# fishaudio/fish-diffusion

Hardware: NVIDIA H100
Metric: mel_frames_per_sec_100step_ddpm (higher is better)
Workload: dtype f32 (3x fp16 split-product wgmma, fp32 accumulate)

## Files before the change

### fish_diffusion_b200/csrc/fd_tapgemm_tc.cu

```cuda
#include <cuda.h>
#include "fd_common.cuh"
#include "fd_host.h"
#include "fd_tc_ptx.cuh"

namespace {

constexpr int BLOCK_M = 128;

constexpr int ring_stages(int stage_bytes, int bias_floats) {
  return fd_tc_ring_stages(1024  + bias_floats * 4 + 2 * FD_TC_MAX_STAGES * 8 + FD_TC_SCRATCH_BYTES,
                           stage_bytes);
}

template <int BLOCK_N, int BLOCK_K, int EPI, int NPL>
struct Cfg {
  static constexpr bool PP = EPI == FD_EPI_GATE || EPI == FD_EPI_RES_SKIP;
  static constexpr int ROWS = PP ? 64 : BLOCK_M;
  static constexpr int A_BYTES = ROWS * BLOCK_K * 2;
  static constexpr int W_BYTES = BLOCK_N * BLOCK_K * 2;
  static constexpr int GROUP = BLOCK_K >= 64 || PP ? 1 : 64 / BLOCK_K;
  static constexpr int SUB_BYTES = NPL * (A_BYTES + W_BYTES);
  static constexpr int STAGE_BYTES = GROUP * SUB_BYTES;
  static constexpr int TX_BYTES = SUB_BYTES;
  static constexpr int SWIZZLE_BYTES = BLOCK_K * 2;
  static constexpr uint32_t SWIZZLE_MODE = swizzle_mode_for(SWIZZLE_BYTES);
  static constexpr uint32_t SBO = 8 * SWIZZLE_BYTES;
  static constexpr int BIAS_FLOATS = (EPI == FD_EPI_GATE ? 3 : 1) * BLOCK_N;
  static constexpr int BIAS_TOTAL = (PP ? 2 : 1) * BIAS_FLOATS;
  static constexpr int NUM_STAGES = ring_stages(STAGE_BYTES, BIAS_TOTAL);
  static constexpr int SMEM_BYTES = 1024  + NUM_STAGES * STAGE_BYTES + BIAS_TOTAL * 4 +
                                    2 * NUM_STAGES * 8 + FD_TC_SCRATCH_BYTES;
  static_assert(NUM_STAGES >= 2, "pipeline needs at least two stages");
  static_assert(SMEM_BYTES <= FD_TC_SMEM_BUDGET, "shared memory");
};

template <int BLOCK_N, int EPI>
__device__ __forceinline__ void stage_bias(const FdTapGemm& p, int b, int n0, float* bias_s, int i0, int step) {
  if (EPI == FD_EPI_GATE) {
    const size_t bo = (size_t)b * p.gbias_bstride + n0;
    for (int i = i0; i < BLOCK_N; i += step) {
      bias_s[i] = p.gbias_full[bo + i];
      bias_s[BLOCK_N + i] = p.gbias_lo[bo + i];
      bias_s[2 * BLOCK_N + i] = p.gbias_hi[bo + i];
    }
  } else {
    for (int i = i0; i < BLOCK_N; i += step)
      bias_s[i] = p.bias ? p.bias[(size_t)b * p.bias_bstride + n0 + i] : 0.f;
  }
}
template <int EPI>
__device__ __forceinline__ long long bias_key(const FdTapGemm& p, int b, int n0) {
  return EPI == FD_EPI_GATE ? (long long)b * p.gbias_bstride + n0 : (long long)b * p.bias_bstride + n0;
}

template <int BLOCK_N, int EPI, int PREC>
__device__ __forceinline__ void tile_epilogue(const FdTapGemm& p, const float* acc, int b, int n_tile, int rw0,
                                              const float* bias_s, uint32_t my_scratch, int lane) {
  const int n0 = n_tile * BLOCK_N;
  if (EPI == FD_EPI_GATE || EPI == FD_EPI_MAG) {
    constexpr int HALF = BLOCK_N / 2;
    const uint32_t sb = smem_u32(bias_s);
    const int r = lane >> 1, sub = lane & 1;
    const int t = rw0 + r;
    const bool valid = t < p.T;
    const bool e_lo = t < p.dil, e_hi = t + p.dil >= p.T;
    const bool edge_any = __any_sync(0xffffffffu, valid && (e_lo || e_hi));
    const size_t zplane = (size_t)p.B * p.T * p.C, zrow = ((size_t)b * p.T + t) * p.C + (size_t)n_tile * HALF;
    const size_t yplane = (size_t)p.B * p.T * p.n_total, yrow = ((size_t)b * p.T + t) * p.n_total;
    const int halfg = p.gate_tile / 2;
#pragma unroll
    for (int c = 0; c < HALF; c += 16) {
      frag_to_scratch<16>(my_scratch, acc, c, 0, lane);
      frag_to_scratch<16>(my_scratch, acc, HALF + c, 16, lane);
      __syncwarp();
      float g[8], f[8];
      {
        const float4 g0 = scratch_ld4(my_scratch, r, 2 * sub), g1 = scratch_ld4(my_scratch, r, 2 * sub + 1);
        const float4 f0 = scratch_ld4(my_scratch, r, 4 + 2 * sub), f1 = scratch_ld4(my_scratch, r, 5 + 2 * sub);
        g[0] = g0.x; g[1] = g0.y; g[2] = g0.z; g[3] = g0.w; g[4] = g1.x; g[5] = g1.y; g[6] = g1.z; g[7] = g1.w;
        f[0] = f0.x; f[1] = f0.y; f[2] = f0.z; f[3] = f0.w; f[4] = f1.x; f[5] = f1.y; f[6] = f1.z; f[7] = f1.w;
      }
      __syncwarp();
      const int cc = c + 8 * sub;
      if (valid) {
        if (EPI == FD_EPI_MAG) {
          fd_epi_mag<8, PREC>(p, b, t, n_tile * HALF + cc, g, f);
        } else {
          float yg[8], yf[8], z[8];
          {
            float4 c0, c1, d0, d1;
            if (p.addend != nullptr) {
              const float* ad = p.addend + yrow + n0 + cc;
              c0 = __ldcs(reinterpret_cast<const float4*>(ad));
              c1 = __ldcs(reinterpret_cast<const float4*>(ad + 4));
              d0 = __ldcs(reinterpret_cast<const float4*>(ad + HALF));
              d1 = __ldcs(reinterpret_cast<const float4*>(ad + HALF + 4));
            }
            const float4 a0 = lds128(sb + 4u * cc), a1 = lds128(sb + 4u * cc + 16u);
            const float4 b0 = lds128(sb + 4u * (HALF + cc)), b1 = lds128(sb + 4u * (HALF + cc) + 16u);
            const float bg[8] = {a0.x, a0.y, a0.z, a0.w, a1.x, a1.y, a1.z, a1.w};
            const float bf[8] = {b0.x, b0.y, b0.z, b0.w, b1.x, b1.y, b1.z, b1.w};
#pragma unroll
            for (int i = 0; i < 8; ++i) {
              yg[i] = g[i] * p.acc_scale + bg[i];
              yf[i] = f[i] * p.acc_scale + bf[i];
            }
            if (p.addend != nullptr) {
              const float cg[8] = {c0.x, c0.y, c0.z, c0.w, c1.x, c1.y, c1.z, c1.w};
              const float cf[8] = {d0.x, d0.y, d0.z, d0.w, d1.x, d1.y, d1.z, d1.w};
#pragma unroll
              for (int i = 0; i < 8; ++i) { yg[i] += cg[i]; yf[i] += cf[i]; }
            }
          }
          if (edge_any) {
#pragma unroll
            for (int e = 0; e < 2; ++e) {
              if (e == 0 ? e_lo : e_hi) {
                const uint32_t eb = sb + 4u * ((1 + e) * BLOCK_N + cc);
                const float4 a0 = lds128(eb), a1 = lds128(eb + 16u);
                const float4 b0 = lds128(eb + 4u * HALF), b1 = lds128(eb + 4u * HALF + 16u);
                const float eg[8] = {a0.x, a0.y, a0.z, a0.w, a1.x, a1.y, a1.z, a1.w};
                const float ef[8] = {b0.x, b0.y, b0.z, b0.w, b1.x, b1.y, b1.z, b1.w};
#pragma unroll
                for (int i = 0; i < 8; ++i) { yg[i] -= eg[i]; yf[i] -= ef[i]; }
              }
            }
          }
#pragma unroll
          for (int i = 0; i < 8; ++i) z[i] = fd_sigmoid(yg[i]) * fd_tanh(yf[i]);
          if (p.y_planes != nullptr) {
            const int zc0 = n_tile * HALF + cc;
            const int ng = p.gate_tile == BLOCK_N ? n_tile * BLOCK_N + cc : (zc0 / halfg) * p.gate_tile + (zc0 % halfg);
            fd_store_planes<8>(p.y_planes, yplane, yrow + ng, yg, PREC);
            fd_store_planes<8>(p.y_planes, yplane, yrow + ng + halfg, yf, PREC);
          }
          fd_store_planes<8>(p.out_planes, zplane, zrow + cc, z, PREC);
        }
      }
    }
  } else if (BLOCK_N >= 64) {
    const uint32_t bias_addr = smem_u32(bias_s);
    const int j4 = (lane & 7) * 4, rsub = lane >> 3;
    const int rbase = rw0 + rsub;
    const int nrows = rbase < p.T ? min(4, (p.T - rbase + 3) / 4) : 0;
    const uint32_t rowbase = (uint32_t)b * (uint32_t)p.T;
#pragma unroll
    for (int c = 0; c < BLOCK_N; c += 32) {
      const int col = c + j4;
      const int n = n0 + col;
      frag_to_scratch<32>(my_scratch, acc, c, 0, lane);
      __syncwarp();
      float4 a[4];
#pragma unroll
      for (int pp = 0; pp < 4; ++pp) a[pp] = scratch_ld4(my_scratch, 4 * pp + rsub, lane & 7);
      __syncwarp();
      if (EPI == FD_EPI_GATE_BWD) {
        const int half_g = p.gate_tile / 2;
        const uint32_t pg = (uint32_t)((n / half_g) * p.gate_tile + (n % half_g));
        const uint32_t W2 = 2u * (uint32_t)p.C;
        const size_t yplane = (size_t)p.B * p.T * W2;
        const uint16_t* const y_lo = p.y_planes + yplane;
        uint16_t* const o_lo = p.out_planes + yplane;
        float sg4[4] = {0.f, 0.f, 0.f, 0.f}, sf4[4] = {0.f, 0.f, 0.f, 0.f};
        float e0g[4] = {0.f, 0.f, 0.f, 0.f}, e0f[4] = {0.f, 0.f, 0.f, 0.f}, e1g[4] = {0.f, 0.f, 0.f, 0.f}, e1f[4] = {0.f, 0.f, 0.f, 0.f};
        uint2 gh[4], gl[4], fh[4], fl[4];
        uint32_t eo4[4];
#pragma unroll
        for (int pp = 0; pp < 4; ++pp) {
          eo4[pp] = (rowbase + (uint32_t)min(rbase + pp * 4, p.T - 1)) * W2 + pg;
          gh[pp] = *reinterpret_cast<const uint2*>(p.y_planes + eo4[pp]);
          gl[pp] = *reinterpret_cast<const uint2*>(y_lo + eo4[pp]);
          fh[pp] = *reinterpret_cast<const uint2*>(p.y_planes + eo4[pp] + half_g);
          fl[pp] = *reinterpret_cast<const uint2*>(y_lo + eo4[pp] + half_g);
        }
#pragma unroll
        for (int pp = 0; pp < 4; ++pp) {
          if (pp >= nrows) break;
          float g[4], f[4];
          fd_combine2(gh[pp].x, gl[pp].x, PREC, g[0], g[1]);
          fd_combine2(gh[pp].y, gl[pp].y, PREC, g[2], g[3]);
          fd_combine2(fh[pp].x, fl[pp].x, PREC, f[0], f[1]);
          fd_combine2(fh[pp].y, fl[pp].y, PREC, f[2], f[3]);
          const float dzv[4] = {a[pp].x * p.acc_scale, a[pp].y * p.acc_scale, a[pp].z * p.acc_scale, a[pp].w * p.acc_scale};
          float dg[4], df[4];
#pragma unroll
          for (int i = 0; i < 4; ++i) fd_dgate(dzv[i], g[i], f[i], dg[i], df[i]);
          uint32_t h0, l0, h1, l1;
          fd_split2(dg[0], dg[1], PREC, h0, l0);
          fd_split2(dg[2], dg[3], PREC, h1, l1);
          *reinterpret_cast<uint2*>(p.out_planes + eo4[pp]) = make_uint2(h0, h1);
          *reinterpret_cast<uint2*>(o_lo + eo4[pp]) = make_uint2(l0, l1);
          fd_split2(df[0], df[1], PREC, h0, l0);
          fd_split2(df[2], df[3], PREC, h1, l1);
          *reinterpret_cast<uint2*>(p.out_planes + eo4[pp] + half_g) = make_uint2(h0, h1);
          *reinterpret_cast<uint2*>(o_lo + eo4[pp] + half_g) = make_uint2(l0, l1);
          if (p.cs != nullptr) {
            const int tt = rbase + pp * 4;
            const bool in0 = tt < p.dil, in1 = tt + p.dil >= p.T;
#pragma unroll
            for (int i = 0; i < 4; ++i) {
              sg4[i] += dg[i]; sf4[i] += df[i];
              if (in0) { e0g[i] += dg[i]; e0f[i] += df[i]; }
              if (in1) { e1g[i] += dg[i]; e1f[i] += df[i]; }
            }
          }
        }
        if (p.cs != nullptr) {
          const bool edge0 = rw0 < p.dil, edge1 = rw0 + 16 + p.dil > p.T;
#pragma unroll
          for (int i = 0; i < 4; ++i) {
            sg4[i] += __shfl_xor_sync(0xffffffffu, sg4[i], 8); sg4[i] += __shfl_xor_sync(0xffffffffu, sg4[i], 16);
            sf4[i] += __shfl_xor_sync(0xffffffffu, sf4[i], 8); sf4[i] += __shfl_xor_sync(0xffffffffu, sf4[i], 16);
            if (edge0) {
              e0g[i] += __shfl_xor_sync(0xffffffffu, e0g[i], 8); e0g[i] += __shfl_xor_sync(0xffffffffu, e0g[i], 16);
              e0f[i] += __shfl_xor_sync(0xffffffffu, e0f[i], 8); e0f[i] += __shfl_xor_sync(0xffffffffu, e0f[i], 16);
            }
            if (edge1) {
              e1g[i] += __shfl_xor_sync(0xffffffffu, e1g[i], 8); e1g[i] += __shfl_xor_sync(0xffffffffu, e1g[i], 16);
              e1f[i] += __shfl_xor_sync(0xffffffffu, e1f[i], 8); e1f[i] += __shfl_xor_sync(0xffffffffu, e1f[i], 16);
            }
          }
          if (rsub == 0) {
            float* const csb = p.cs + (size_t)b * W2 + pg;
#pragma unroll
            for (int i = 0; i < 4; ++i) {
              atomicAdd(csb + i, sg4[i] * p.cs_scale);
              atomicAdd(csb + half_g + i, sf4[i] * p.cs_scale);
            }
            if (p.cs_edge != nullptr && (edge0 || edge1)) {
              float* const ce0 = p.cs_edge + (size_t)b * W2 + pg;
              float* const ce1 = ce0 + (size_t)p.B * W2;
#pragma unroll
              for (int i = 0; i < 4; ++i) {
                if (edge0) { atomicAdd(ce0 + i, e0g[i] * p.cs_scale); atomicAdd(ce0 + half_g + i, e0f[i] * p.cs_scale); }
                if (edge1) { atomicAdd(ce1 + i, e1g[i] * p.cs_scale); atomicAdd(ce1 + half_g + i, e1f[i] * p.cs_scale); }
              }
            }
          }
        }
      } else if (EPI == FD_EPI_RES_SKIP) {
        const float4 bias4 = lds128(bias_addr + 4u * col);
        const bool is_res = n0 < p.C;
        const uint32_t cn = (uint32_t)(is_res ? n : n - p.C);
        const size_t plane = (size_t)p.B * p.T * p.C;
        uint32_t eo[4];
#pragma unroll
        for (int pp = 0; pp < 4; ++pp)
          eo[pp] = (rowbase + (uint32_t)min(rbase + pp * 4, p.T - 1)) * (uint32_t)p.C + cn;
        if (is_res) {
          if (!p.last_layer) {
            const uint16_t* const xlo = p.x_planes + plane;
            uint16_t* const xo = p.x_out_planes != nullptr ? p.x_out_planes : p.x_planes;
            uint16_t* const xo_lo = xo + plane;
            uint2 h2[4], l2[4];
#pragma unroll
            for (int pp = 0; pp < 4; ++pp) {
              h2[pp] = *reinterpret_cast<const uint2*>(p.x_planes + eo[pp]);
              l2[pp] = *reinterpret_cast<const uint2*>(xlo + eo[pp]);
            }
#pragma unroll
            for (int pp = 0; pp < 4; ++pp) {
              if (pp >= nrows) break;
              float x0, x1, x2, x3;
              fd_combine2(h2[pp].x, l2[pp].x, PREC, x0, x1);
              fd_combine2(h2[pp].y, l2[pp].y, PREC, x2, x3);
              x0 = (x0 + (a[pp].x * p.acc_scale + bias4.x)) * 0.70710678118654752440f;
              x1 = (x1 + (a[pp].y * p.acc_scale + bias4.y)) * 0.70710678118654752440f;
              x2 = (x2 + (a[pp].z * p.acc_scale + bias4.z)) * 0.70710678118654752440f;
              x3 = (x3 + (a[pp].w * p.acc_scale + bias4.w)) * 0.70710678118654752440f;
              uint32_t h0, l0, h1, l1;
              fd_split2(x0, x1, PREC, h0, l0);
              fd_split2(x2, x3, PREC, h1, l1);
              *reinterpret_cast<uint2*>(xo + eo[pp]) = make_uint2(h0, h1);
              *reinterpret_cast<uint2*>(xo_lo + eo[pp]) = make_uint2(l0, l1);
            }
          }
        } else {
          float4 sk[4];
          if (!p.first_layer) {
#pragma unroll
            for (int pp = 0; pp < 4; ++pp) sk[pp] = *reinterpret_cast<const float4*>(p.skip_f32 + eo[pp]);
          }
          uint16_t* const sk_lo = p.skip_planes + plane;
#pragma unroll
          for (int pp = 0; pp < 4; ++pp) {
            if (pp >= nrows) break;
            float y0 = a[pp].x * p.acc_scale + bias4.x, y1 = a[pp].y * p.acc_scale + bias4.y;
            float y2 = a[pp].z * p.acc_scale + bias4.z, y3 = a[pp].w * p.acc_scale + bias4.w;
            if (!p.first_layer) { y0 += sk[pp].x; y1 += sk[pp].y; y2 += sk[pp].z; y3 += sk[pp].w; }
            if (p.last_layer) {
              uint32_t h0, l0, h1, l1;
              fd_split2(y0 * p.skip_scale, y1 * p.skip_scale, PREC, h0, l0);
              fd_split2(y2 * p.skip_scale, y3 * p.skip_scale, PREC, h1, l1);
              *reinterpret_cast<uint2*>(p.skip_planes + eo[pp]) = make_uint2(h0, h1);
              *reinterpret_cast<uint2*>(sk_lo + eo[pp]) = make_uint2(l0, l1);
            } else {
              *reinterpret_cast<float4*>(p.skip_f32 + eo[pp]) = make_float4(y0, y1, y2, y3);
            }
          }
        }
      } else {
        const float4 bias4 = lds128(bias_addr + 4u * col);
        uint32_t eo[4];
#pragma unroll
        for (int pp = 0; pp < 4; ++pp)
          eo[pp] = (rowbase + (uint32_t)min(rbase + pp * 4, p.T - 1)) * (uint32_t)p.n_total + (uint32_t)n;
        float4 pre[4];
#pragma unroll
        for (int pp = 0; pp < 4; ++pp) pre[pp] = make_float4(0.f, 0.f, 0.f, 0.f);
        if (p.addend != nullptr) {
#pragma unroll
          for (int pp = 0; pp < 4; ++pp) {
            const float4 t4 = *reinterpret_cast<const float4*>(p.addend + eo[pp]);
            pre[pp].x += t4.x; pre[pp].y += t4.y; pre[pp].z += t4.z; pre[pp].w += t4.w;
          }
        }
        if (p.res_f32 != nullptr) {
#pragma unroll
          for (int pp = 0; pp < 4; ++pp) {
            const float4 t4 = *reinterpret_cast<const float4*>(p.res_f32 + eo[pp]);
            pre[pp].x += t4.x; pre[pp].y += t4.y; pre[pp].z += t4.z; pre[pp].w += t4.w;
          }
        }
        if (p.res_planes != nullptr) {
          const uint16_t* const lo_base = p.res_planes + (size_t)p.B * p.T * p.n_total;
#pragma unroll
          for (int pp = 0; pp < 4; ++pp) {
            const uint2 h2 = *reinterpret_cast<const uint2*>(p.res_planes + eo[pp]);
            const uint2 l2 = *reinterpret_cast<const uint2*>(lo_base + eo[pp]);
            float r0, r1, r2, r3;
            fd_combine2(h2.x, l2.x, PREC, r0, r1);
            fd_combine2(h2.y, l2.y, PREC, r2, r3);
            pre[pp].x += p.res_scale * r0; pre[pp].y += p.res_scale * r1;
            pre[pp].z += p.res_scale * r2; pre[pp].w += p.res_scale * r3;
          }
        }
        uint32_t mkbits = 0;
        if (p.row_mask != nullptr) {
#pragma unroll
          for (int pp = 0; pp < 4; ++pp)
            if (p.row_mask[rowbase + (uint32_t)min(rbase + pp * 4, p.T - 1)] != 0) mkbits |= 1u << pp;
        }
#pragma unroll
        for (int pp = 0; pp < 4; ++pp) {
          a[pp].x = (a[pp].x * p.acc_scale + bias4.x + pre[pp].x) * p.post_scale;
          a[pp].y = (a[pp].y * p.acc_scale + bias4.y + pre[pp].y) * p.post_scale;
          a[pp].z = (a[pp].z * p.acc_scale + bias4.z + pre[pp].z) * p.post_scale;
          a[pp].w = (a[pp].w * p.acc_scale + bias4.w + pre[pp].w) * p.post_scale;
        }
        if (p.out_f32 != nullptr && p.out_accum) {
#pragma unroll
          for (int pp = 0; pp < 4; ++pp) {
            const float4 o4 = *reinterpret_cast<const float4*>(p.out_f32 + eo[pp]);
            a[pp].x += o4.x; a[pp].y += o4.y; a[pp].z += o4.z; a[pp].w += o4.w;
          }
        }
        const float slope = p.act == FD_ACT_NONE ? 1.f : p.act == FD_ACT_RELU ? 0.f : p.act_slope;
        uint16_t* const out_lo = p.out_planes + (size_t)p.B * p.T * p.n_total;
#pragma unroll
        for (int pp = 0; pp < 4; ++pp) {
          if (pp >= nrows) break;
          if ((mkbits >> pp) & 1u) a[pp] = make_float4(0.f, 0.f, 0.f, 0.f);
          if (p.out_f32 != nullptr) *reinterpret_cast<float4*>(p.out_f32 + eo[pp]) = a[pp];
          if (p.out_planes != nullptr) {
            uint32_t h0, l0, h1, l1;
            fd_split2(fd_act(a[pp].x * p.planes_scale, slope), fd_act(a[pp].y * p.planes_scale, slope), PREC, h0, l0);
            fd_split2(fd_act(a[pp].z * p.planes_scale, slope), fd_act(a[pp].w * p.planes_scale, slope), PREC, h1, l1);
            *reinterpret_cast<uint2*>(p.out_planes + eo[pp]) = make_uint2(h0, h1);
            *reinterpret_cast<uint2*>(out_lo + eo[pp]) = make_uint2(l0, l1);
          }
        }
      }
    }
  } else {
    constexpr int PER = BLOCK_N / 2;
    frag_to_scratch<BLOCK_N>(my_scratch, acc, 0, 0, lane);
    __syncwarp();
    const int r = lane >> 1, sub = lane & 1;
    float v[PER];
#pragma unroll
    for (int q4 = 0; q4 < PER / 4; ++q4) {
      const float4 x = scratch_ld4(my_scratch, r, sub * (PER / 4) + q4);
      v[4 * q4] = x.x; v[4 * q4 + 1] = x.y; v[4 * q4 + 2] = x.z; v[4 * q4 + 3] = x.w;
    }
    __syncwarp();
    const int t = rw0 + r;
    if (t < p.T) {
#pragma unroll
      for (int h = 0; h < PER / 8; ++h) {
        float v8[8];
#pragma unroll
        for (int i = 0; i < 8; ++i) v8[i] = v[h * 8 + i];
        const int cc = sub * PER + h * 8;
        if (EPI == FD_EPI_LINEAR) fd_epi_linear<8, PREC>(p, b, t, n0 + cc, v8, bias_s, n0);
        else fd_epi_res_skip<8, PREC>(p, b, t, n0 + cc, v8, bias_s + cc);
      }
    }
  }
}

template <int BLOCK_N, int BLOCK_K, int EPI, int PREC, int NPL>
__global__ void __launch_bounds__(FD_TC_THREADS, 1)
fd_tapgemm_tc_kernel(const __grid_constant__ CUtensorMap tm_src0, const __grid_constant__ CUtensorMap tm_src1,
                     const __grid_constant__ CUtensorMap tm_w, const FdTapGemm p) {
  using C = Cfg<BLOCK_N, BLOCK_K, EPI, NPL>;
  static_assert(!C::PP, "GATE / RES_SKIP run the ping-pong schedule");
  using MMA = Wgmma<BLOCK_N, PREC>;
  extern __shared__ uint8_t smem_raw[];
  uint8_t* smem = reinterpret_cast<uint8_t*>((reinterpret_cast<uintptr_t>(smem_raw) + 1023) & ~(uintptr_t)1023);
  uint8_t* stage_base = smem;
  float* bias_s = reinterpret_cast<float*>(smem + C::NUM_STAGES * C::STAGE_BYTES);
  uint64_t* full_bar = reinterpret_cast<uint64_t*>(bias_s + C::BIAS_TOTAL);
  uint64_t* empty_bar = full_bar + C::NUM_STAGES;
  float* scratch_s = reinterpret_cast<float*>(empty_bar + C::NUM_STAGES);

  const int warp = threadIdx.x / 32;
  const int lane = threadIdx.x % 32;

  const int tiles_t = (p.T + BLOCK_M - 1) / BLOCK_M;
  const int num_m_tiles = p.B * tiles_t;
  const int num_n_tiles = p.n_total / BLOCK_N;
  const int num_tiles = num_m_tiles * num_n_tiles;
  int total_k_blocks = 0;
  for (int sI = 0; sI < p.num_seg; ++sI) total_k_blocks += p.seg[sI].k_len / BLOCK_K;

  if (threadIdx.x == 0) {
    for (int i = 0; i < C::NUM_STAGES; ++i) { mbar_init(&full_bar[i], 1); mbar_init(&empty_bar[i], FD_TC_CONSUMER_THREADS / 32); }
    fence_barrier_init();
  }
  if (warp == FD_TC_PRODUCER_WARP && lane == 0) {
    prefetch_tmap(&tm_src0);
    prefetch_tmap(&tm_src1);
    prefetch_tmap(&tm_w);
  }
  __syncthreads();

  if (warp >= FD_TC_PRODUCER_WARP) {
    producer_regs();
    if (warp == FD_TC_PRODUCER_WARP && lane == 0) {
      int stage = 0; uint32_t phase = 0;
      for (int tile = blockIdx.x; tile < num_tiles; tile += gridDim.x) {
        const int m_tile = tile / num_n_tiles;
        const int n_tile = (tile % num_n_tiles + m_tile) % num_n_tiles;
        const int b = m_tile / tiles_t, t0 = (m_tile % tiles_t) * BLOCK_M;
        const int n0 = n_tile * BLOCK_N;
        int s = 0, k0 = 0, koff = 0;
        for (int kb = 0; kb < total_k_blocks; kb += C::GROUP) {
          const int nb = min(C::GROUP, total_k_blocks - kb);
          mbar_wait(&empty_bar[stage], phase ^ 1);
          uint8_t* st = stage_base + stage * C::STAGE_BYTES;
          mbar_expect_tx(&full_bar[stage], nb * C::TX_BYTES);
          for (int g = 0; g < nb; ++g) {
            const FdSeg sg = p.seg[s];
            const CUtensorMap* tm = sg.src == 0 ? &tm_src0 : &tm_src1;
            uint8_t* sub = st + g * C::SUB_BYTES;
            tma_load_4d(sub, tm, &full_bar[stage], sg.c_off + k0, t0 + sg.shift, b, 0);
            const int kw = koff + k0 + p.w_kshift;
            tma_load_3d(sub + NPL * C::A_BYTES, &tm_w, &full_bar[stage], kw, n0, 0);
            k0 += BLOCK_K;
            if (k0 >= sg.k_len) { koff += sg.k_len; k0 = 0; ++s; }
          }
          if (++stage == C::NUM_STAGES) { stage = 0; phase ^= 1; }
        }
      }
    }
    return;
  }

  consumer_regs();
  const int wg = warp / 4;
  const int wq = warp % 4;
  const uint32_t my_scratch = smem_u32(scratch_s) + warp * FD_TC_SCRATCH_WARP_BYTES;
  float acc[BLOCK_N / 2];
  int stage = 0; uint32_t phase = 0;
  long long staged_key = -1;
  for (int tile = blockIdx.x; tile < num_tiles; tile += gridDim.x) {
    const int m_tile = tile / num_n_tiles;
    const int n_tile = (tile % num_n_tiles + m_tile) % num_n_tiles;
    const int b = m_tile / tiles_t, t0 = (m_tile % tiles_t) * BLOCK_M;
    const int n0 = n_tile * BLOCK_N;

    if (EPI == FD_EPI_LINEAR && bias_key<EPI>(p, b, n0) != staged_key) {
      staged_key = bias_key<EPI>(p, b, n0);
      asm volatile("bar.sync 1, %0;" ::"r"(FD_TC_CONSUMER_THREADS) : "memory");
      stage_bias<BLOCK_N, EPI>(p, b, n0, bias_s, threadIdx.x, FD_TC_CONSUMER_THREADS);
      asm volatile("bar.sync 1, %0;" ::"r"(FD_TC_CONSUMER_THREADS) : "memory");
    }

#pragma unroll
    for (int i = 0; i < BLOCK_N / 2; ++i) acc[i] = 0.f;
    int prev_stage = -1;
    for (int kb = 0; kb < total_k_blocks; kb += C::GROUP) {
      const int nb = min(C::GROUP, total_k_blocks - kb);
      mbar_wait(&full_bar[stage], phase);
      wg_fence_operand(acc);
      wg_fence();
      for (int g = 0; g < nb; ++g) {
        const uint32_t st = smem_u32(stage_base + stage * C::STAGE_BYTES + g * C::SUB_BYTES);
        const uint32_t wg_a = wg * 64 * C::SWIZZLE_BYTES;
        const uint64_t a_hi = make_smem_desc(st + wg_a, 16, C::SBO, C::SWIZZLE_MODE);
        const uint64_t a_lo = make_smem_desc(st + C::A_BYTES + wg_a, 16, C::SBO, C::SWIZZLE_MODE);
        const uint64_t w_hi = make_smem_desc(st + NPL * C::A_BYTES, 16, C::SBO, C::SWIZZLE_MODE);
        const uint64_t w_lo = make_smem_desc(st + NPL * C::A_BYTES + C::W_BYTES, 16, C::SBO, C::SWIZZLE_MODE);
#pragma unroll
        for (int k = 0; k < BLOCK_K / 16; ++k) {
          const uint64_t adv = (uint64_t)((k * 32) >> 4);
          if (NPL == 2) {
            MMA::template ss<0, 0>(acc, a_lo + adv, w_hi + adv, 1u);
            MMA::template ss<0, 0>(acc, a_hi + adv, w_lo + adv, 1u);
            MMA::template ss<0, 0>(acc, a_hi + adv, w_hi + adv, 1u);
          } else {
            MMA::template ss<0, 0>(acc, a_hi + adv, w_hi + adv, 1u);
          }
        }
      }
      wg_commit();
      wg_wait<1>();
      wg_fence_operand(acc);
      if (prev_stage >= 0 && lane == 0) mbar_arrive(&empty_bar[prev_stage]);
      prev_stage = stage;
      if (++stage == C::NUM_STAGES) { stage = 0; phase ^= 1; }
    }
    wg_wait<0>();
    wg_fence_operand(acc);
    if (prev_stage >= 0 && lane == 0) mbar_arrive(&empty_bar[prev_stage]);

    tile_epilogue<BLOCK_N, EPI, PREC>(p, acc, b, n_tile, t0 + wg * 64 + wq * 16, bias_s, my_scratch, lane);
  }
}

template <int BLOCK_N, int BLOCK_K, int EPI, int PREC, int NPL>
__global__ void __launch_bounds__(FD_TC_THREADS, 1)
fd_tapgemm_pp_kernel(const __grid_constant__ CUtensorMap tm_src0, const __grid_constant__ CUtensorMap tm_src1,
                     const __grid_constant__ CUtensorMap tm_w, const FdTapGemm p) {
  using C = Cfg<BLOCK_N, BLOCK_K, EPI, NPL>;
  static_assert(C::PP && C::GROUP == 1, "ping-pong schedule: GATE / RES_SKIP, one k-block per stage");
  using MMA = Wgmma<BLOCK_N, PREC>;
  extern __shared__ uint8_t smem_raw[];
  uint8_t* smem = reinterpret_cast<uint8_t*>((reinterpret_cast<uintptr_t>(smem_raw) + 1023) & ~(uintptr_t)1023);
  uint8_t* stage_base = smem;
  float* bias_s = reinterpret_cast<float*>(smem + C::NUM_STAGES * C::STAGE_BYTES);
  uint64_t* full_bar = reinterpret_cast<uint64_t*>(bias_s + C::BIAS_TOTAL);
  uint64_t* empty_bar = full_bar + C::NUM_STAGES;
  float* scratch_s = reinterpret_cast<float*>(empty_bar + C::NUM_STAGES);

  const int warp = threadIdx.x / 32;
  const int lane = threadIdx.x % 32;
  const int rank = (int)cluster_ctarank();
  const int pair = blockIdx.x / 2, num_pairs = gridDim.x / 2;

  const int tiles_t = (p.T + 63) / 64;
  const int num_m_tiles = p.B * tiles_t;
  const int num_n_tiles = p.n_total / BLOCK_N;
  const int num_units = (num_m_tiles + 1) / 2 * num_n_tiles;
  int total_k_blocks = 0;
  for (int sI = 0; sI < p.num_seg; ++sI) total_k_blocks += p.seg[sI].k_len / BLOCK_K;

  if (threadIdx.x == 0) {
    for (int i = 0; i < C::NUM_STAGES; ++i) { mbar_init(&full_bar[i], 1); mbar_init(&empty_bar[i], 2 * 4); }
    fence_barrier_init();
  }
  if (warp == FD_TC_PRODUCER_WARP && lane == 0) {
    prefetch_tmap(&tm_src0);
    prefetch_tmap(&tm_src1);
    prefetch_tmap(&tm_w);
  }
  cluster_sync();

  if (warp >= FD_TC_PRODUCER_WARP) {
    producer_regs();
    if (warp == FD_TC_PRODUCER_WARP && lane == 0) {
      int stage = 0; uint32_t phase = 0;
      for (int u = pair; u < num_units; u += num_pairs) {
        const int m_pair = u / num_n_tiles;
        const int n_tile = (u % num_n_tiles + m_pair) % num_n_tiles;
        const int m_tile = min(2 * m_pair + rank, num_m_tiles - 1);
        const int b = m_tile / tiles_t, t0 = (m_tile % tiles_t) * 64;
        const int n0 = n_tile * BLOCK_N;
        int s = 0, k0 = 0, koff = 0;
#pragma unroll 1
        for (int kb = 0; kb < total_k_blocks; ++kb) {
          mbar_wait(&empty_bar[stage], phase ^ 1);
          uint8_t* st = stage_base + stage * C::STAGE_BYTES;
          mbar_expect_tx(&full_bar[stage], C::TX_BYTES);
          const FdSeg sg = p.seg[s];
          tma_load_4d(st, sg.src == 0 ? &tm_src0 : &tm_src1, &full_bar[stage], sg.c_off + k0, t0 + sg.shift, b, 0);
          tma_load_3d_multicast(st + NPL * C::A_BYTES + rank * (NPL * C::W_BYTES / 2), &tm_w, &full_bar[stage],
                                koff + k0 + p.w_kshift, n0 + (NPL == 1 ? rank * (BLOCK_N / 2) : 0),
                                NPL == 2 ? rank : 0, 0x3);
          k0 += BLOCK_K;
          if (k0 >= sg.k_len) { koff += sg.k_len; k0 = 0; ++s; }
          if (++stage == C::NUM_STAGES) { stage = 0; phase ^= 1; }
        }
      }
    }
  } else {
    consumer_regs();
    const int wg = warp / 4;
    const int wq = warp % 4;
    const uint32_t my_scratch = smem_u32(scratch_s) + warp * FD_TC_SCRATCH_WARP_BYTES;
    float* my_bias = bias_s + wg * C::BIAS_FLOATS;
    float acc[BLOCK_N / 2];
    int stage = 0; uint32_t phase = 0;
    auto advance = [&](int n) {
      stage += n;
      phase ^= (uint32_t)(stage / C::NUM_STAGES) & 1u;
      stage %= C::NUM_STAGES;
    };
    auto release = [&](int st) {
      if (lane == 0) { mbar_arrive_cluster(&empty_bar[st], 0); mbar_arrive_cluster(&empty_bar[st], 1); }
    };
    if (wg == 1) advance(total_k_blocks);
    long long staged_key = -1;
    for (int u = pair + wg * num_pairs; u < num_units; u += 2 * num_pairs) {
      const int m_pair = u / num_n_tiles;
      const int n_tile = (u % num_n_tiles + m_pair) % num_n_tiles;
      const int m_tile = 2 * m_pair + rank;
      const bool valid = m_tile < num_m_tiles;
      const int b = m_tile / tiles_t, t0 = (m_tile % tiles_t) * 64;
      const int n0 = n_tile * BLOCK_N;

      if (valid && bias_key<EPI>(p, b, n0) != staged_key) {
        staged_key = bias_key<EPI>(p, b, n0);
        wg == 0 ? named_bar_sync<3, 128>() : named_bar_sync<4, 128>();
        stage_bias<BLOCK_N, EPI>(p, b, n0, my_bias, threadIdx.x % 128, 128);
        wg == 0 ? named_bar_sync<3, 128>() : named_bar_sync<4, 128>();
      }

      if (u != pair) wg == 0 ? named_bar_sync<1, 256>() : named_bar_sync<2, 256>();
      const bool pass = u + num_pairs < num_units;
#pragma unroll
      for (int i = 0; i < BLOCK_N / 2; ++i) acc[i] = 0.f;
      int prev_stage = -1;
      for (int kb = 0; kb < total_k_blocks; ++kb) {
        mbar_wait(&full_bar[stage], phase);
        wg_fence_operand(acc);
        wg_fence();
        const uint32_t st = smem_u32(stage_base + stage * C::STAGE_BYTES);
        const uint64_t a_hi = make_smem_desc(st, 16, C::SBO, C::SWIZZLE_MODE);
        const uint64_t a_lo = make_smem_desc(st + C::A_BYTES, 16, C::SBO, C::SWIZZLE_MODE);
        const uint64_t w_hi = make_smem_desc(st + NPL * C::A_BYTES, 16, C::SBO, C::SWIZZLE_MODE);
        const uint64_t w_lo = make_smem_desc(st + NPL * C::A_BYTES + C::W_BYTES, 16, C::SBO, C::SWIZZLE_MODE);
#pragma unroll
        for (int k = 0; k < BLOCK_K / 16; ++k) {
          const uint64_t adv = (uint64_t)((k * 32) >> 4);
          if (NPL == 2) {
            MMA::template ss<0, 0>(acc, a_lo + adv, w_hi + adv, 1u);
            MMA::template ss<0, 0>(acc, a_hi + adv, w_lo + adv, 1u);
            MMA::template ss<0, 0>(acc, a_hi + adv, w_hi + adv, 1u);
          } else {
            MMA::template ss<0, 0>(acc, a_hi + adv, w_hi + adv, 1u);
          }
        }
        wg_commit();
        if (kb == total_k_blocks - 1 && pass)
          wg == 0 ? named_bar_arrive<2, 256>() : named_bar_arrive<1, 256>();
        wg_wait<1>();
        wg_fence_operand(acc);
        if (prev_stage >= 0) release(prev_stage);
        prev_stage = stage;
        advance(1);
      }
      wg_wait<0>();
      wg_fence_operand(acc);
      if (prev_stage >= 0) release(prev_stage);
      advance(total_k_blocks);

      if (valid) tile_epilogue<BLOCK_N, EPI, PREC>(p, acc, b, n_tile, t0 + wq * 16, my_bias, my_scratch, lane);
    }
  }
  __syncwarp();
  cluster_sync();
}

template <int BLOCK_T>
struct GateTCfg {
  static constexpr int BLOCK_K = 32;
  static constexpr int ROW_BYTES = BLOCK_K * 2;
  static constexpr int ACT_ROWS = BLOCK_T + 16;
  static constexpr int MAX_DIL = (ACT_ROWS - BLOCK_T) / 2;
  static constexpr int ACT_PLANE = ACT_ROWS * ROW_BYTES;
  static constexpr int W_PLANE = 64 * ROW_BYTES;
  static constexpr int W_OFF = 2 * ACT_PLANE;
  static constexpr int STAGE_BYTES = W_OFF + 3 * 2 * W_PLANE;
  static constexpr uint32_t SWIZZLE_MODE = swizzle_mode_for(ROW_BYTES);
  static constexpr uint32_t SBO = 8 * ROW_BYTES;
  static constexpr int NUM_STAGES =
      fd_tc_ring_stages(1024  + 2 * FD_TC_MAX_STAGES * 8 + FD_TC_SCRATCH_BYTES, STAGE_BYTES);
  static constexpr int SMEM_BYTES = 1024 + NUM_STAGES * STAGE_BYTES + 2 * NUM_STAGES * 8 + FD_TC_SCRATCH_BYTES;
  static_assert(ACT_ROWS <= 256, "one TMA box per plane");
  static_assert(ACT_PLANE % 512 == 0 && STAGE_BYTES % 1024 == 0, "planes start on 64 B swizzle atoms");
  static_assert(NUM_STAGES >= 3, "ring depth");
  static_assert(SMEM_BYTES <= FD_TC_SMEM_BUDGET, "shared memory");
};

template <int BLOCK_T, int PREC>
__device__ __forceinline__ void gate_t_epilogue(const FdTapGemm& p, const float* acc, int b, int t0, int ch,
                                                uint32_t my_scratch, int lane) {
  const int half = p.gate_tile / 2;
  const int e = lane >> 2, q4 = lane & 3;
  const int n_g = (ch / half) * p.gate_tile + ch % half + e, n_f = n_g + half;
  const size_t bo = (size_t)b * p.gbias_bstride;
  const float bg = p.gbias_full[bo + n_g], bf = p.gbias_full[bo + n_f];
  const float lg = p.gbias_lo[bo + n_g], lf = p.gbias_lo[bo + n_f];
  const float hg = p.gbias_hi[bo + n_g], hf = p.gbias_hi[bo + n_f];
  const size_t row0 = (size_t)b * p.T;
  const size_t zplane = (size_t)p.B * p.T * p.C;
  constexpr int NG = BLOCK_T / 8;
  auto load_addend = [&](int c0, float (&a)[16]) {
#pragma unroll
    for (int i = 0; i < 16; ++i) a[i] = 0.f;
    if (p.addend == nullptr) return;
#pragma unroll
    for (int ci = 0; ci < 4; ++ci) {
      if (c0 + ci < NG) {
#pragma unroll
        for (int s = 0; s < 2; ++s) {
          const int t = min(t0 + 8 * (c0 + ci) + 2 * q4 + s, p.T - 1);
          const float* ad = p.addend + (row0 + t) * p.n_total;
          a[4 * ci + 2 * s] = __ldcs(ad + n_g);
          a[4 * ci + 2 * s + 1] = __ldcs(ad + n_f);
        }
      }
    }
  };
  float a_next[16];
  load_addend(0, a_next);
#pragma unroll
  for (int c0 = 0; c0 < NG; c0 += 4) {
    float a_cur[16];
#pragma unroll
    for (int i = 0; i < 16; ++i) a_cur[i] = a_next[i];
    if (c0 + 4 < NG) load_addend(c0 + 4, a_next);
#pragma unroll
    for (int ci = 0; ci < 4; ++ci) {
      if (c0 + ci < NG) {
#pragma unroll
        for (int s = 0; s < 2; ++s) {
          const int tl = 8 * ci + 2 * q4 + s;
          const int t = t0 + 8 * c0 + tl;
          float yg = acc[4 * (c0 + ci) + s] * p.acc_scale + bg + a_cur[4 * ci + 2 * s];
          float yf = acc[4 * (c0 + ci) + 2 + s] * p.acc_scale + bf + a_cur[4 * ci + 2 * s + 1];
          if (t < p.dil) { yg -= lg; yf -= lf; }
          if (t + p.dil >= p.T) { yg -= hg; yf -= hf; }
          sts32(my_scratch + 4u * (tl * 8 + (((e >> 2) ^ ((tl >> 2) & 1)) << 2) + (e & 3)),
                fd_sigmoid(yg) * fd_tanh(yf));
        }
      }
    }
    __syncwarp();
    const int t = t0 + 8 * c0 + lane;
    if (lane < 8 * min(4, NG - c0) && t < p.T) {
      const uint32_t sw = (uint32_t)((lane >> 2) & 1);
      const float4 z0 = lds128(my_scratch + 4u * (lane * 8 + (sw << 2)));
      const float4 z1 = lds128(my_scratch + 4u * (lane * 8 + ((sw ^ 1u) << 2)));
      const float z[8] = {z0.x, z0.y, z0.z, z0.w, z1.x, z1.y, z1.z, z1.w};
      fd_store_planes<8>(p.out_planes, zplane, (row0 + t) * p.C + ch, z, PREC);
    }
    __syncwarp();
  }
}

template <int BLOCK_T, int PREC>
__global__ void __launch_bounds__(FD_TC_THREADS, 1)
fd_gate_t_kernel(const __grid_constant__ CUtensorMap tm_x, const __grid_constant__ CUtensorMap tm_w, const FdTapGemm p) {
  using C = GateTCfg<BLOCK_T>;
  using MMA = Wgmma<BLOCK_T, PREC>;
  extern __shared__ uint8_t smem_raw[];
  uint8_t* smem = reinterpret_cast<uint8_t*>((reinterpret_cast<uintptr_t>(smem_raw) + 1023) & ~(uintptr_t)1023);
  uint8_t* stage_base = smem;
  uint64_t* full_bar = reinterpret_cast<uint64_t*>(smem + C::NUM_STAGES * C::STAGE_BYTES);
  uint64_t* empty_bar = full_bar + C::NUM_STAGES;
  float* scratch_s = reinterpret_cast<float*>(empty_bar + C::NUM_STAGES);

  const int warp = threadIdx.x / 32;
  const int lane = threadIdx.x % 32;
  const int rank = (int)cluster_ctarank();
  const int pair = blockIdx.x / 2, num_pairs = gridDim.x / 2;

  const int d = p.dil;
  const int tiles_t = (p.T + BLOCK_T - 1) / BLOCK_T;
  const int num_wp = p.n_total / 128;
  const int num_units = p.B * tiles_t * num_wp;
  const int k_blocks = p.C / C::BLOCK_K;

  if (threadIdx.x == 0) {
    for (int i = 0; i < C::NUM_STAGES; ++i) { mbar_init(&full_bar[i], 1); mbar_init(&empty_bar[i], 2 * 4); }
    fence_barrier_init();
  }
  if (warp == FD_TC_PRODUCER_WARP && lane == 0) {
    prefetch_tmap(&tm_x);
    prefetch_tmap(&tm_w);
  }
  cluster_sync();

  if (warp >= FD_TC_PRODUCER_WARP) {
    producer_regs();
    if (warp == FD_TC_PRODUCER_WARP && lane == 0) {
      const uint32_t tx = 2u * (uint32_t)(BLOCK_T + 2 * d) * C::ROW_BYTES + 3 * 2 * C::W_PLANE;
      const int half = p.gate_tile / 2;
      int stage = 0; uint32_t phase = 0;
      for (int u = pair; u < num_units; u += num_pairs) {
        const int tt = u / num_wp, wt = 2 * (u % num_wp) + rank;
        const int b = tt / tiles_t, t0 = (tt % tiles_t) * BLOCK_T;
        const int ch = wt * 32;
        const int g0 = ((ch / half) * p.gate_tile + ch % half) / 8;
#pragma unroll 1
        for (int kb = 0; kb < k_blocks; ++kb) {
          mbar_wait(&empty_bar[stage], phase ^ 1);
          uint8_t* st = stage_base + stage * C::STAGE_BYTES;
          mbar_expect_tx(&full_bar[stage], tx);
          tma_load_4d_multicast(st + rank * C::ACT_PLANE, &tm_x, &full_bar[stage], kb * C::BLOCK_K, t0 - d, b, rank,
                                0x3);
#pragma unroll 1
          for (int j = 0; j < 3; ++j)
            tma_load_5d(st + C::W_OFF + j * 2 * C::W_PLANE, &tm_w, &full_bar[stage], j * p.C + kb * C::BLOCK_K, 0, 0,
                        g0, 0);
          if (++stage == C::NUM_STAGES) { stage = 0; phase ^= 1; }
        }
      }
    }
  } else {
    consumer_regs();
    const int wg = warp / 4;
    const int wq = warp % 4;
    const uint32_t my_scratch = smem_u32(scratch_s) + warp * FD_TC_SCRATCH_WARP_BYTES;
    float acc[BLOCK_T / 2];
    int stage = 0; uint32_t phase = 0;
    auto advance = [&](int n) {
      stage += n;
      phase ^= (uint32_t)(stage / C::NUM_STAGES) & 1u;
      stage %= C::NUM_STAGES;
    };
    auto release = [&](int st) {
      if (lane == 0) { mbar_arrive_cluster(&empty_bar[st], 0); mbar_arrive_cluster(&empty_bar[st], 1); }
    };
    if (wg == 1) advance(k_blocks);
    for (int u = pair + wg * num_pairs; u < num_units; u += 2 * num_pairs) {
      const int tt = u / num_wp, wt = 2 * (u % num_wp) + rank;
      const int b = tt / tiles_t, t0 = (tt % tiles_t) * BLOCK_T;

      if (u != pair) wg == 0 ? named_bar_sync<1, 256>() : named_bar_sync<2, 256>();
      const bool pass = u + num_pairs < num_units;
#pragma unroll
      for (int i = 0; i < BLOCK_T / 2; ++i) acc[i] = 0.f;
      int prev_stage = -1;
      for (int kb = 0; kb < k_blocks; ++kb) {
        mbar_wait(&full_bar[stage], phase);
        wg_fence_operand(acc);
        wg_fence();
        const uint32_t st = smem_u32(stage_base + stage * C::STAGE_BYTES);
#pragma unroll
        for (int j = 0; j < 3; ++j) {
          const uint32_t xa = st + (uint32_t)(j * d * C::ROW_BYTES);
          const uint64_t x_hi = make_smem_desc(xa, 16, C::SBO, C::SWIZZLE_MODE);
          const uint64_t x_lo = make_smem_desc(xa + C::ACT_PLANE, 16, C::SBO, C::SWIZZLE_MODE);
          const uint32_t wa = st + C::W_OFF + j * 2 * C::W_PLANE;
          const uint64_t w_hi = make_smem_desc(wa, 16, C::SBO, C::SWIZZLE_MODE);
          const uint64_t w_lo = make_smem_desc(wa + C::W_PLANE, 16, C::SBO, C::SWIZZLE_MODE);
#pragma unroll
          for (int k = 0; k < C::BLOCK_K / 16; ++k) {
            const uint64_t adv = (uint64_t)((k * 32) >> 4);
            MMA::template ss<0, 0>(acc, w_hi + adv, x_lo + adv, 1u);
            MMA::template ss<0, 0>(acc, w_lo + adv, x_hi + adv, 1u);
            MMA::template ss<0, 0>(acc, w_hi + adv, x_hi + adv, 1u);
          }
        }
        wg_commit();
        if (kb == k_blocks - 1 && pass) wg == 0 ? named_bar_arrive<2, 256>() : named_bar_arrive<1, 256>();
        wg_wait<1>();
        wg_fence_operand(acc);
        if (prev_stage >= 0) release(prev_stage);
        prev_stage = stage;
        advance(1);
      }
      wg_wait<0>();
      wg_fence_operand(acc);
      if (prev_stage >= 0) release(prev_stage);
      advance(k_blocks);

      gate_t_epilogue<BLOCK_T, PREC>(p, acc, b, t0, wt * 32 + wq * 8, my_scratch, lane);
    }
  }
  __syncwarp();
  cluster_sync();
}

int gate_t_block(const FdTapGemm& p) {
  if (p.epi != FD_EPI_GATE || p.single || p.y_planes != nullptr || p.num_seg != 3 || p.w_kshift != 0) return 0;
  if (p.C % GateTCfg<200>::BLOCK_K != 0 || p.n_total != 2 * p.C || p.src_C[0] != p.C) return 0;
  if ((p.gate_tile != 256 && p.gate_tile != 128) || p.n_total % p.gate_tile != 0) return 0;
  for (int s = 0; s < 3; ++s)
    if (p.seg[s].src != 0 || p.seg[s].shift != (s - 1) * p.dil || p.seg[s].c_off != 0 || p.seg[s].k_len != p.C)
      return 0;
  int best = 0;
  long long best_pad = 0;
  for (const int bt : {200, 240}) {
    if (p.dil > (bt == 200 ? GateTCfg<200>::MAX_DIL : GateTCfg<240>::MAX_DIL)) continue;
    const long long pad = (long long)(p.T + bt - 1) / bt * bt;
    if (best == 0 || pad < best_pad || (pad == best_pad && bt > best)) { best = bt; best_pad = pad; }
  }
  return best;
}

template <int BLOCK_T, int PREC>
int launch_gate_t(const FdTapGemm& p, cudaStream_t stream) {
  using C = GateTCfg<BLOCK_T>;
  CUtensorMap tmx, tmw;
  int rc = planes_map(&tmx, p.src[0], p.src_C[0], p.T, p.B, p.src_rs[0], p.src_bs[0], p.src_ps[0], C::BLOCK_K,
                      BLOCK_T + 2 * p.dil, 1, "gate_t x");
  if (rc) return rc;
  const int half = p.gate_tile / 2;
  const cuuint64_t K = (cuuint64_t)p.k_total;
  const cuuint64_t dims[5] = {K, 8, 2, (cuuint64_t)p.n_total / 8, 2};
  const cuuint64_t strides[4] = {K * 2, (cuuint64_t)half * K * 2, 8 * K * 2, (cuuint64_t)p.n_total * K * 2};
  const cuuint32_t box[5] = {(cuuint32_t)C::BLOCK_K, 8, 2, 4, 2};
  rc = encode_tiled(&tmw, p.w, 5, dims, strides, box, "gate_t w");
  if (rc) return rc;
  const int units = p.B * ((p.T + BLOCK_T - 1) / BLOCK_T) * (p.n_total / 128);
  return fd_tc_launch<fd_gate_t_kernel<BLOCK_T, PREC>>(C::SMEM_BYTES, 2 * units, stream, false, 2, tmx, tmw, p);
}

template <int BLOCK_N, int BLOCK_K, int EPI, int PREC, int NPL>
int launch_inst(const FdTapGemm& p, cudaStream_t stream) {
  using C = Cfg<BLOCK_N, BLOCK_K, EPI, NPL>;
  CUtensorMap tm0, tm1, tmw;
  int rc = planes_map(&tm0, p.src[0], p.src_C[0], p.T, p.B, p.src_rs[0], p.src_bs[0], p.src_ps[0], BLOCK_K, C::ROWS,
                      NPL, "tapgemm src0");
  if (rc) return rc;
  if (p.src[1] != nullptr) {
    rc = planes_map(&tm1, p.src[1], p.src_C[1], p.T, p.B, p.src_rs[1], p.src_bs[1], p.src_ps[1], BLOCK_K, C::ROWS, NPL,
                    "tapgemm src1");
    if (rc) return rc;
  } else {
    tm1 = tm0;
  }
  const int m_tiles = p.B * ((p.T + C::ROWS - 1) / C::ROWS), n_tiles = p.n_total / BLOCK_N;
  if constexpr (C::PP) {
    rc = weights_map(&tmw, p.w, p.n_total, p.k_total, BLOCK_K, NPL == 2 ? BLOCK_N : BLOCK_N / 2, 1, "tapgemm w");
    if (rc) return rc;
    return fd_tc_launch<fd_tapgemm_pp_kernel<BLOCK_N, BLOCK_K, EPI, PREC, NPL>>(
        C::SMEM_BYTES, 2 * ((m_tiles + 1) / 2 * n_tiles), stream, false, 2, tm0, tm1, tmw, p);
  } else {
    rc = weights_map(&tmw, p.w, p.n_total, p.k_total, BLOCK_K, BLOCK_N, NPL, "tapgemm w");
    if (rc) return rc;
    return fd_tc_launch<fd_tapgemm_tc_kernel<BLOCK_N, BLOCK_K, EPI, PREC, NPL>>(C::SMEM_BYTES, m_tiles * n_tiles,
                                                                              stream, false, 1, tm0, tm1, tmw, p);
  }
}

template <int BLOCK_N, int BLOCK_K, int EPI>
int launch_cfg(const FdTapGemm& p, cudaStream_t stream) {
  if (p.single) {
    return p.prec == FD_F16 ? launch_inst<BLOCK_N, BLOCK_K, EPI, FD_F16, 1>(p, stream)
                            : launch_inst<BLOCK_N, BLOCK_K, EPI, FD_BF16, 1>(p, stream);
  }
  return p.prec == FD_F16 ? launch_inst<BLOCK_N, BLOCK_K, EPI, FD_F16, 2>(p, stream)
                          : launch_inst<BLOCK_N, BLOCK_K, EPI, FD_BF16, 2>(p, stream);
}

template <int BLOCK_N, int BLOCK_K>
int launch_epi(const FdTapGemm& p, cudaStream_t stream) {
  if (p.epi == FD_EPI_GATE) return launch_cfg<BLOCK_N, BLOCK_K, FD_EPI_GATE>(p, stream);
  if (p.epi == FD_EPI_MAG) return launch_cfg<BLOCK_N, BLOCK_K, FD_EPI_MAG>(p, stream);
  if (p.epi == FD_EPI_RES_SKIP) return launch_cfg<BLOCK_N, BLOCK_K, FD_EPI_RES_SKIP>(p, stream);
  if (p.epi == FD_EPI_GATE_BWD) return launch_cfg<BLOCK_N, BLOCK_K, FD_EPI_GATE_BWD>(p, stream);
  return launch_cfg<BLOCK_N, BLOCK_K, FD_EPI_LINEAR>(p, stream);
}

void pick_cfg(const FdTapGemm& p, int* bn, int* bk) {
  *bn = 0; *bk = 0;
// ... 85 lines not shown
```

Measured before the change: 22840.

## Prefetch residual/skip epilogue operands before the MMA loop in ping-pong kernel

Adds a dedicated RES_SKIP epilogue for the ping-pong tap-GEMM when BLOCK_N >= 64. Before the wgmma k-loop it computes row offsets and issues the first chunk's residual-plane or skip loads, so their latency is hidden behind the MMAs. Later chunks are software-pipelined: the next chunk is loaded while the current one is processed. Loads use __ldcg and stores use streaming __stcs hints. The cost is extra registers held across the MMA loop, which may reduce occupancy or cause spills, and a static_assert now restricts the old path to BLOCK_N <= 32.

```diff
diff --git a/fish_diffusion_b200/csrc/fd_tapgemm_tc.cu b/fish_diffusion_b200/csrc/fd_tapgemm_tc.cu
--- a/fish_diffusion_b200/csrc/fd_tapgemm_tc.cu
+++ b/fish_diffusion_b200/csrc/fd_tapgemm_tc.cu
@@ -56,6 +56,7 @@
 template <int BLOCK_N, int EPI, int PREC>
 __device__ __forceinline__ void tile_epilogue(const FdTapGemm& p, const float* acc, int b, int n_tile, int rw0,
                                               const float* bias_s, uint32_t my_scratch, int lane) {
+  static_assert(EPI != FD_EPI_RES_SKIP || BLOCK_N <= 32, "RES_SKIP with coalescing tiles: res_skip_epilogue");
   const int n0 = n_tile * BLOCK_N;
   if (EPI == FD_EPI_GATE || EPI == FD_EPI_MAG) {
     constexpr int HALF = BLOCK_N / 2;
@@ -238,67 +239,6 @@
             }
           }
         }
-      } else if (EPI == FD_EPI_RES_SKIP) {
-        const float4 bias4 = lds128(bias_addr + 4u * col);
-        const bool is_res = n0 < p.C;
-        const uint32_t cn = (uint32_t)(is_res ? n : n - p.C);
-        const size_t plane = (size_t)p.B * p.T * p.C;
-        uint32_t eo[4];
-#pragma unroll
-        for (int pp = 0; pp < 4; ++pp)
-          eo[pp] = (rowbase + (uint32_t)min(rbase + pp * 4, p.T - 1)) * (uint32_t)p.C + cn;
-        if (is_res) {
-          if (!p.last_layer) {
-            const uint16_t* const xlo = p.x_planes + plane;
-            uint16_t* const xo = p.x_out_planes != nullptr ? p.x_out_planes : p.x_planes;
-            uint16_t* const xo_lo = xo + plane;
-            uint2 h2[4], l2[4];
-#pragma unroll
-            for (int pp = 0; pp < 4; ++pp) {
-              h2[pp] = *reinterpret_cast<const uint2*>(p.x_planes + eo[pp]);
-              l2[pp] = *reinterpret_cast<const uint2*>(xlo + eo[pp]);
-            }
-#pragma unroll
-            for (int pp = 0; pp < 4; ++pp) {
-              if (pp >= nrows) break;
-              float x0, x1, x2, x3;
-              fd_combine2(h2[pp].x, l2[pp].x, PREC, x0, x1);
-              fd_combine2(h2[pp].y, l2[pp].y, PREC, x2, x3);
-              x0 = (x0 + (a[pp].x * p.acc_scale + bias4.x)) * 0.70710678118654752440f;
-              x1 = (x1 + (a[pp].y * p.acc_scale + bias4.y)) * 0.70710678118654752440f;
-              x2 = (x2 + (a[pp].z * p.acc_scale + bias4.z)) * 0.70710678118654752440f;
-              x3 = (x3 + (a[pp].w * p.acc_scale + bias4.w)) * 0.70710678118654752440f;
-              uint32_t h0, l0, h1, l1;
-              fd_split2(x0, x1, PREC, h0, l0);
-              fd_split2(x2, x3, PREC, h1, l1);
-              *reinterpret_cast<uint2*>(xo + eo[pp]) = make_uint2(h0, h1);
-              *reinterpret_cast<uint2*>(xo_lo + eo[pp]) = make_uint2(l0, l1);
-            }
-          }
-        } else {
-          float4 sk[4];
-          if (!p.first_layer) {
-#pragma unroll
-            for (int pp = 0; pp < 4; ++pp) sk[pp] = *reinterpret_cast<const float4*>(p.skip_f32 + eo[pp]);
-          }
-          uint16_t* const sk_lo = p.skip_planes + plane;
-#pragma unroll
-          for (int pp = 0; pp < 4; ++pp) {
-            if (pp >= nrows) break;
-            float y0 = a[pp].x * p.acc_scale + bias4.x, y1 = a[pp].y * p.acc_scale + bias4.y;
-            float y2 = a[pp].z * p.acc_scale + bias4.z, y3 = a[pp].w * p.acc_scale + bias4.w;
-            if (!p.first_layer) { y0 += sk[pp].x; y1 += sk[pp].y; y2 += sk[pp].z; y3 += sk[pp].w; }
-            if (p.last_layer) {
-              uint32_t h0, l0, h1, l1;
-              fd_split2(y0 * p.skip_scale, y1 * p.skip_scale, PREC, h0, l0);
-              fd_split2(y2 * p.skip_scale, y3 * p.skip_scale, PREC, h1, l1);
-              *reinterpret_cast<uint2*>(p.skip_planes + eo[pp]) = make_uint2(h0, h1);
-              *reinterpret_cast<uint2*>(sk_lo + eo[pp]) = make_uint2(l0, l1);
-            } else {
-              *reinterpret_cast<float4*>(p.skip_f32 + eo[pp]) = make_float4(y0, y1, y2, y3);
-            }
-          }
-        }
       } else {
         const float4 bias4 = lds128(bias_addr + 4u * col);
         uint32_t eo[4];
@@ -396,6 +336,120 @@
         else fd_epi_res_skip<8, PREC>(p, b, t, n0 + cc, v8, bias_s + cc);
       }
     }
+  }
+}
+
+struct ResSkipRows {
+  uint32_t eo[4];
+  int nrows;
+  bool is_res;
+  bool loads;
+  bool active;
+};
+
+template <int BLOCK_N>
+__device__ __forceinline__ ResSkipRows res_skip_rows(const FdTapGemm& p, int b, int n_tile, int rw0, int lane) {
+  ResSkipRows r;
+  const int n0 = n_tile * BLOCK_N;
+  const int rbase = rw0 + (lane >> 3);
+  r.nrows = rbase < p.T ? min(4, (p.T - rbase + 3) / 4) : 0;
+  r.is_res = n0 < p.C;
+  r.loads = r.is_res ? !p.last_layer : !p.first_layer;
+  r.active = !(r.is_res && p.last_layer);
+  const uint32_t rowbase = (uint32_t)b * (uint32_t)p.T;
+  const uint32_t cn = (uint32_t)((r.is_res ? n0 : n0 - p.C) + (lane & 7) * 4);
+#pragma unroll
+  for (int pp = 0; pp < 4; ++pp) r.eo[pp] = (rowbase + (uint32_t)min(rbase + pp * 4, p.T - 1)) * (uint32_t)p.C + cn;
+  return r;
+}
+
+__device__ __forceinline__ void res_skip_load(const FdTapGemm& p, const ResSkipRows& r, int c, uint4 (&v)[4]) {
+  if (!r.loads) return;
+  if (r.is_res) {
+    const uint16_t* const xlo = p.x_planes + (size_t)p.B * p.T * p.C;
+#pragma unroll
+    for (int pp = 0; pp < 4; ++pp) {
+      const uint2 h = __ldcg(reinterpret_cast<const uint2*>(p.x_planes + r.eo[pp] + c));
+      const uint2 l = __ldcg(reinterpret_cast<const uint2*>(xlo + r.eo[pp] + c));
+      v[pp] = make_uint4(h.x, h.y, l.x, l.y);
+    }
+  } else {
+#pragma unroll
+    for (int pp = 0; pp < 4; ++pp) {
+      const float4 s = __ldcg(reinterpret_cast<const float4*>(p.skip_f32 + r.eo[pp] + c));
+      v[pp] = make_uint4(__float_as_uint(s.x), __float_as_uint(s.y), __float_as_uint(s.z), __float_as_uint(s.w));
+    }
+  }
+}
+
+template <int BLOCK_N, int PREC>
+__device__ __forceinline__ void res_skip_epilogue(const FdTapGemm& p, const float* acc, const ResSkipRows& r,
+                                                  uint4 (&next)[4], const float* bias_s, uint32_t my_scratch, int lane) {
+  if (!r.active) return;
+  const uint32_t bias_addr = smem_u32(bias_s);
+  const int j4 = (lane & 7) * 4, rsub = lane >> 3;
+  const size_t plane = (size_t)p.B * p.T * p.C;
+  uint16_t* const xo = p.x_out_planes != nullptr ? p.x_out_planes : p.x_planes;
+  uint16_t* const xo_lo = xo + plane;
+  uint16_t* const sk_lo = p.skip_planes + plane;
+  constexpr int NCH = BLOCK_N / 32;
+  auto chunk_col = [](int k) { return 32 * (k < NCH / 2 ? 2 * k : 2 * (k - NCH / 2) + 1); };
+#pragma unroll
+  for (int k = 0; k < NCH; ++k) {
+    const int c = chunk_col(k);
+    const bool late = NCH == 2 && k == 0 && r.is_res;
+    uint4 v[4];
+#pragma unroll
+    for (int pp = 0; pp < 4; ++pp) v[pp] = next[pp];
+    if (k + 1 < NCH && !late) res_skip_load(p, r, chunk_col(k + 1), next);
+    frag_to_scratch<32>(my_scratch, acc, c, 0, lane);
+    __syncwarp();
+    float4 a[4];
+#pragma unroll
+    for (int pp = 0; pp < 4; ++pp) a[pp] = scratch_ld4(my_scratch, 4 * pp + rsub, lane & 7);
+    __syncwarp();
+    const float4 bias4 = lds128(bias_addr + 4u * (c + j4));
+    if (r.is_res) {
+#pragma unroll
+      for (int pp = 0; pp < 4; ++pp) {
+        if (pp >= r.nrows) break;
+        const uint32_t o = r.eo[pp] + c;
+        float x0, x1, x2, x3;
+        fd_combine2(v[pp].x, v[pp].z, PREC, x0, x1);
+        fd_combine2(v[pp].y, v[pp].w, PREC, x2, x3);
+        x0 = (x0 + (a[pp].x * p.acc_scale + bias4.x)) * 0.70710678118654752440f;
+        x1 = (x1 + (a[pp].y * p.acc_scale + bias4.y)) * 0.70710678118654752440f;
+        x2 = (x2 + (a[pp].z * p.acc_scale + bias4.z)) * 0.70710678118654752440f;
+        x3 = (x3 + (a[pp].w * p.acc_scale + bias4.w)) * 0.70710678118654752440f;
+        uint32_t h0, l0, h1, l1;
+        fd_split2(x0, x1, PREC, h0, l0);
+        fd_split2(x2, x3, PREC, h1, l1);
+        __stcs(reinterpret_cast<uint2*>(xo + o), make_uint2(h0, h1));
+        __stcs(reinterpret_cast<uint2*>(xo_lo + o), make_uint2(l0, l1));
+      }
+    } else {
+#pragma unroll
+      for (int pp = 0; pp < 4; ++pp) {
+        if (pp >= r.nrows) break;
+        const uint32_t o = r.eo[pp] + c;
+        float y0 = a[pp].x * p.acc_scale + bias4.x, y1 = a[pp].y * p.acc_scale + bias4.y;
+        float y2 = a[pp].z * p.acc_scale + bias4.z, y3 = a[pp].w * p.acc_scale + bias4.w;
+        if (!p.first_layer) {
+          y0 += __uint_as_float(v[pp].x); y1 += __uint_as_float(v[pp].y);
+          y2 += __uint_as_float(v[pp].z); y3 += __uint_as_float(v[pp].w);
+        }
+        if (p.last_layer) {
+          uint32_t h0, l0, h1, l1;
+          fd_split2(y0 * p.skip_scale, y1 * p.skip_scale, PREC, h0, l0);
+          fd_split2(y2 * p.skip_scale, y3 * p.skip_scale, PREC, h1, l1);
+          __stcs(reinterpret_cast<uint2*>(p.skip_planes + o), make_uint2(h0, h1));
+          __stcs(reinterpret_cast<uint2*>(sk_lo + o), make_uint2(l0, l1));
+        } else {
+          __stcs(reinterpret_cast<float4*>(p.skip_f32 + o), make_float4(y0, y1, y2, y3));
+        }
+      }
+    }
+    if (late) res_skip_load(p, r, chunk_col(k + 1), next);
   }
 }
 
@@ -627,6 +681,14 @@
         wg == 0 ? named_bar_sync<3, 128>() : named_bar_sync<4, 128>();
       }
 
+      constexpr bool RS = EPI == FD_EPI_RES_SKIP && BLOCK_N >= 64;
+      ResSkipRows rs;
+      uint4 rs_next[4];
+      if constexpr (RS) {
+        rs = res_skip_rows<BLOCK_N>(p, b, n_tile, t0 + wq * 16, lane);
+        if (valid) res_skip_load(p, rs, 0, rs_next);
+      }
+
       if (u != pair) wg == 0 ? named_bar_sync<1, 256>() : named_bar_sync<2, 256>();
       const bool pass = u + num_pairs < num_units;
 #pragma unroll
@@ -666,7 +728,12 @@
       if (prev_stage >= 0) release(prev_stage);
       advance(total_k_blocks);
 
-      if (valid) tile_epilogue<BLOCK_N, EPI, PREC>(p, acc, b, n_tile, t0 + wq * 16, my_bias, my_scratch, lane);
+      if (valid) {
+        if constexpr (RS)
+          res_skip_epilogue<BLOCK_N, PREC>(p, acc, rs, rs_next, my_bias, my_scratch, lane);
+        else
+          tile_epilogue<BLOCK_N, EPI, PREC>(p, acc, b, n_tile, t0 + wq * 16, my_bias, my_scratch, lane);
+      }
     }
   }
   __syncwarp();
```

New measurement: 23250 (median of 6 runs). +1.8%, better.
